# chaofengc/FeMaSR

Hardware: AMD Instinct MI355X
Metric: SR output megapixels/sec at x4 (128->512) (higher is better)
Workload: dtype f32 (1x1 convs / nn.Linear: every fp32 operand split EXACTLY into three bf16 terms, six partial products, fp32 accumulation on the bf16 matrix pipe - closer to fp64 than the fp32 fmaf chain, bit-identical to the CPU oracle)

## Files before the change

femasr_amd/csrc/kernels_misc.hip:

```cpp
#include "common.h"
#include "detmath.h"
#include <stdlib.h>
#include <string.h>

namespace {

__device__ __forceinline__ float4 ld4(const float *p) { return *reinterpret_cast<const float4 *>(p); }

__device__ __forceinline__ int xcd_remap_misc(int bid, int nblk)
{
    const int q = nblk >> 3, r = nblk & 7, xcd = bid & 7, within = bid >> 3;
    return (xcd < r ? xcd * (q + 1) : r * (q + 1) + (xcd - r) * q) + within;
}

__global__ void pad_nchw_to_nhwc_kernel(const float *__restrict__ in, int B, int C, int H, int W, int Hp, int Wp,
                                        float *__restrict__ out, size_t total)
{
    for (size_t i = blockIdx.x * (size_t)blockDim.x + threadIdx.x; i < total; i += (size_t)gridDim.x * blockDim.x) {
        const int c = (int)(i % C);
        size_t r = i / C;
        const int x = (int)(r % Wp);
        r /= Wp;
        const int y = (int)(r % Hp);
        const int n = (int)(r / Hp);
// ... 148 lines not shown
    const int slabs = C >> 5, cg = C >> 5;
    int b = blockIdx.x;
    const int slab = b % slabs;
    b /= slabs;
    const int tx = b % tilesX;
    b /= tilesX;
    const int ty = b % tilesY;
    const int n = b / tilesY;
    const float *xn = x + (size_t)n * H * W * C + slab * 32 + c31;
    double S = 0.0, SS = 0.0;
#pragma unroll
    for (int q = 0; q < 4; ++q) {
        double s = 0.0, ss = 0.0;
#pragma unroll
        for (int r = 0; r < 16; ++r) {
            const int m = 32 * q + 4 * h + (r & 3) + 8 * (r >> 2);
            const int y = 8 * ty + (m >> 4), xx = 16 * tx + (m & 15);
            if (y < H && xx < W) {
                const double d = (double)xn[((size_t)y * W + xx) * C];
                s = s + d;
                ss = __builtin_fma(d, d, ss);
            }
        }
        s = s + __shfl_xor(s, 32, 64);
        ss = ss + __shfl_xor(ss, 32, 64);
        for (int d = 1; d < cg; d <<= 1) {
            s = s + __shfl_xor(s, d, 64);
            ss = ss + __shfl_xor(ss, d, 64);
        }
        if (q == 0) { S = s; SS = ss; } else { S = S + s; SS = SS + ss; }
    }
    const int ch = slab * 32 + c31;
    if (lane < 32 && (ch & (cg - 1)) == 0) {
        double *dst = part + ((((size_t)n * tilesY + ty) * tilesX + tx) * 32 + ch / cg) * 2;
        dst[0] = S;
        dst[1] = SS;
    }
}

__global__ __launch_bounds__(64) void gn_finalize_partials_kernel(const double *__restrict__ part, int tiles, int H, int W, int C, int G,
                                                                  const float *__restrict__ gamma, const float *__restrict__ beta,
                                                                  float eps, float *__restrict__ a, float *__restrict__ b)
{
    const int n = blockIdx.x / G, g = blockIdx.x % G, lane = threadIdx.x, cg = C / G;
    const double *src = part + ((size_t)n * tiles * G + g) * 2;
    double S = 0.0, SS = 0.0;
    for (int t = lane; t < tiles; t += 64) {
        S += src[(size_t)t * G * 2];
        SS += src[(size_t)t * G * 2 + 1];
    }
#pragma unroll
    for (int sft = 32; sft >= 1; sft >>= 1) {
        S += __shfl_xor(S, sft, 64);
        SS += __shfl_xor(SS, sft, 64);
    }
    const double N = (double)H * (double)W * (double)cg;
    const double mean = S / N;
    double var = SS / N - mean * mean;
    if (var < 0.0) var = 0.0;
    const float rstd = 1.0f / sqrtf((float)var + eps);
    const float meanf = (float)mean;
    if (lane < cg) {
        const int c = g * cg + lane;
        const float ac = rstd * gamma[c];
        a[n * C + c] = ac;
        b[n * C + c] = __builtin_fmaf(-meanf, ac, beta[c]);
    }
}

__global__ void gn_silu_apply_kernel(const float *__restrict__ x, int C, long long hw, const float *__restrict__ a, const float *__restrict__ b,
                                     float *__restrict__ y, size_t total4)
{
    const int c4n = C >> 2;
    for (size_t i = blockIdx.x * (size_t)blockDim.x + threadIdx.x; i < total4; i += (size_t)gridDim.x * blockDim.x) {
        const int c4 = (int)(i % c4n);
        const size_t n = (i / c4n) / (size_t)hw;
        const float4 v = ld4(x + 4 * i), ga = ld4(a + n * C + 4 * c4), gb = ld4(b + n * C + 4 * c4);
        float4 o;
        o.x = det_silu(__builtin_fmaf(v.x, ga.x, gb.x));
        o.y = det_silu(__builtin_fmaf(v.y, ga.y, gb.y));
        o.z = det_silu(__builtin_fmaf(v.z, ga.z, gb.z));
        o.w = det_silu(__builtin_fmaf(v.w, ga.w, gb.w));
        *reinterpret_cast<float4 *>(y + 4 * i) = o;
    }
}

__device__ __forceinline__ float wave_tree_sum(float p)
{
#pragma unroll
    for (int s = 32; s >= 1; s >>= 1) p = p + __shfl_xor(p, s, 64);
    return p;
}

__global__ void ln_stats_kernel(const float *__restrict__ x, long long rows, float eps, float *__restrict__ stats)
{
    const long long row = (long long)blockIdx.x * (blockDim.x >> 6) + (threadIdx.x >> 6);
    if (row >= rows) return;
    const int lane = threadIdx.x & 63;
    const float4 v = ld4(x + row * 256 + lane * 4);
    float s = v.x;
    s = s + v.y;
    s = s + v.z;
    s = s + v.w;
    const float mean = wave_tree_sum(s) * (1.0f / 256.0f);
    float d = v.x - mean;
    float q = d * d;
    d = v.y - mean;
    q = __builtin_fmaf(d, d, q);
    d = v.z - mean;
    q = __builtin_fmaf(d, d, q);
    d = v.w - mean;
    q = __builtin_fmaf(d, d, q);
    const float var = wave_tree_sum(q) * (1.0f / 256.0f);
    if (lane == 0) {
        stats[2 * row] = mean;
        stats[2 * row + 1] = 1.0f / sqrtf(var + eps);
    }
}

__global__ void layernorm_kernel(const float *__restrict__ x, long long rows, const float *__restrict__ gamma,
                                 const float *__restrict__ beta, float eps, float *__restrict__ y)
{
    const long long row = (long long)blockIdx.x * (blockDim.x >> 6) + (threadIdx.x >> 6);
    if (row >= rows) return;
    const int lane = threadIdx.x & 63;
    const float4 v = ld4(x + row * 256 + lane * 4);
    float s = v.x;
    s = s + v.y;
    s = s + v.z;
    s = s + v.w;
    const float mean = wave_tree_sum(s) * (1.0f / 256.0f);
    float d = v.x - mean;
    float q = d * d;
    d = v.y - mean;
    q = __builtin_fmaf(d, d, q);
    d = v.z - mean;
    q = __builtin_fmaf(d, d, q);
    d = v.w - mean;
    q = __builtin_fmaf(d, d, q);
    const float var = wave_tree_sum(q) * (1.0f / 256.0f);
    const float rstd = 1.0f / sqrtf(var + eps);
    const float4 g = ld4(gamma + lane * 4), b = ld4(beta + lane * 4);
    float4 o;
    o.x = __builtin_fmaf((v.x - mean) * rstd, g.x, b.x);
    o.y = __builtin_fmaf((v.y - mean) * rstd, g.y, b.y);
    o.z = __builtin_fmaf((v.z - mean) * rstd, g.z, b.z);
    o.w = __builtin_fmaf((v.w - mean) * rstd, g.w, b.w);
    *reinterpret_cast<float4 *>(y + row * 256 + lane * 4) = o;
}

constexpr int ATT_HD = 32, ATT_N = 64;
typedef float att_f32x16 __attribute__((ext_vector_type(16)));

template <int UNITS>
__global__ __launch_bounds__(64, 2) void window_attention_reg_kernel(const float *__restrict__ qkv, int B, int H, int W, int C,
                                                                     int heads, int shift, const float *__restrict__ table,
                                                                     float *__restrict__ out, int total)
{
    __shared__ float Ts[UNITS][232];
    const int lane = threadIdx.x, c = lane & 31, hf = lane >> 5;
    const int nwx = W >> 3, nwy = H >> 3;
    struct Unit { int h, wx, wy, n; };
    auto unit_of = [&](int bid) {
        Unit g;
        g.h = bid % heads;
        bid /= heads;
        g.wx = bid % nwx;
        bid /= nwx;
        g.wy = bid % nwy;
        g.n = bid / nwy;
        return g;
    };
    Unit gs[UNITS];
    bool has[UNITS];
#pragma unroll
    for (int u = 0; u < UNITS; ++u) {
        const int bid = (int)blockIdx.x * UNITS + u;
        has[u] = bid < total;
        gs[u] = unit_of(has[u] ? bid : total - 1);
        for (int i = lane; i < 225; i += 64) Ts[u][i] = table[i * heads + gs[u].h];
    }
    const float scale = 0.17677669529663687f;
    auto rowtok = [&](const Unit &g, int iy) { int y = g.wy * 8 + iy + shift; if (y >= H) y -= H; return y * W; };
    auto coltok = [&](const Unit &g, int ix) { int x = g.wx * 8 + ix + shift; if (x >= W) x -= W; return x; };
    auto qb = [&](const Unit &g) { return qkv + (size_t)g.n * H * W * 3 * C + g.h * ATT_HD; };

    float ak[2][16], bq[2][16];
    auto load_qk = [&](const Unit &g) {
        const float *qbase = qb(g);
#pragma unroll
        for (int tI = 0; tI < 2; ++tI) {
            const int w = 32 * tI + c;
            const unsigned tok = (unsigned)(rowtok(g, w >> 3) + coltok(g, w & 7));
            const float *kp = qbase + tok * (unsigned)(3 * C) + C, *qp = qbase + tok * (unsigned)(3 * C);
#pragma unroll
            for (int d4 = 0; d4 < 8; ++d4) {
                const float4 kv = ld4(kp + 4 * d4), qv = ld4(qp + 4 * d4);
                ak[tI][2 * d4] = hf ? kv.y : kv.x;
                ak[tI][2 * d4 + 1] = hf ? kv.w : kv.z;
                bq[tI][2 * d4] = (hf ? qv.y : qv.x) * scale;
                bq[tI][2 * d4 + 1] = (hf ? qv.w : qv.z) * scale;
            }
        }
    };
    load_qk(gs[0]);
#pragma unroll
    for (int u = 0; u < UNITS; ++u) {
        if (!has[u]) break;
        const Unit g = gs[u];
        const float *qbase = qb(g);
        float *obase = out + (size_t)g.n * H * W * C + g.h * ATT_HD;
        const bool masked = shift > 0 && (g.wy == nwy - 1 || g.wx == nwx - 1);
        att_f32x16 sc[2][2];
#pragma unroll
        for (int tj = 0; tj < 2; ++tj)
#pragma unroll
            for (int ti = 0; ti < 2; ++ti)
#pragma unroll
                for (int r = 0; r < 16; ++r) sc[tj][ti][r] = 0.f;
#pragma unroll
        for (int st = 0; st < 16; ++st)
#pragma unroll
            for (int tj = 0; tj < 2; ++tj)
#pragma unroll
                for (int ti = 0; ti < 2; ++ti) sc[tj][ti] = __builtin_amdgcn_mfma_f32_32x32x2f32(ak[tj][st], bq[ti][st], sc[tj][ti], 0, 0, 0);

        float vf[2][16];
        {
            const float *vb = qbase + 2 * C + c;
            unsigned cto[4];
#pragma unroll
            for (int e = 0; e < 4; ++e) cto[e] = (unsigned)coltok(g, e + 4 * hf) * (unsigned)(3 * C);
#pragma unroll
            for (int tj = 0; tj < 2; ++tj)
#pragma unroll
                for (int r = 0; r < 16; ++r) {
                    const unsigned ro = (unsigned)__builtin_amdgcn_readfirstlane(rowtok(g, (r >> 2) + 4 * tj)) * (unsigned)(3 * C);
                    vf[tj][r] = vb[ro + cto[r & 3]];
                }
        }
        if (u + 1 < UNITS && has[u + 1 < UNITS ? u + 1 : u]) load_qk(gs[u + 1 < UNITS ? u + 1 : u]);
#pragma unroll
        for (int ti = 0; ti < 2; ++ti) {
            const int i = 32 * ti + c, iy = i >> 3, ix = i & 7;
            const int tb = (iy + 7) * 15 + ix + 7 - 4 * hf;
            unsigned rowdiff = 0, coldiff = 0;
            if (masked) {
                const int ysi = g.wy * 8 + iy, xsi = g.wx * 8 + ix;
                const int ryi = ysi < H - 8 ? 0 : (ysi < H - shift ? 1 : 2), rxi = xsi < W - 8 ? 0 : (xsi < W - shift ? 1 : 2);
#pragma unroll
                for (int q = 0; q < 8; ++q) {
                    const int ysj = g.wy * 8 + q, xsj = g.wx * 8 + q;
                    const int ryj = ysj < H - 8 ? 0 : (ysj < H - shift ? 1 : 2), rxj = xsj < W - 8 ? 0 : (xsj < W - shift ? 1 : 2);
                    rowdiff |= (ryj != ryi ? 1u : 0u) << q;
                    coldiff |= (rxj != rxi ? 1u : 0u) << q;
                }
                coldiff >>= 4 * hf;
            }
            float m = -INFINITY;
#pragma unroll
            for (int tj = 0; tj < 2; ++tj)
#pragma unroll
                for (int r = 0; r < 16; ++r) {
                    const int jy = (r >> 2) + 4 * tj, jxl = r & 3;
                    float a1 = sc[tj][ti][r] + Ts[u][tb - 15 * jy - jxl];
                    if (masked) a1 = a1 + ((((rowdiff >> jy) | (coldiff >> jxl)) & 1u) ? -100.0f : 0.0f);
                    sc[tj][ti][r] = a1;
                    m = a1 > m ? a1 : m;
                }
            {
                const float mo = __shfl_xor(m, 32, 64);
                m = mo > m ? mo : m;
            }
            float part = 0.f;
#pragma unroll
            for (int tj = 0; tj < 2; ++tj)
#pragma unroll
                for (int r = 0; r < 16; r += 2) {
                    const det_f32x2 e = det_expf2(det_f32x2{sc[tj][ti][r] - m, sc[tj][ti][r + 1] - m});
                    sc[tj][ti][r] = e[0];
                    sc[tj][ti][r + 1] = e[1];
                    part = part + e[0];
                    part = part + e[1];
                }
            const float other = __shfl_xor(part, 32, 64);
            const float rinv = 1.0f / (hf ? other + part : part + other);
#pragma unroll
            for (int tj = 0; tj < 2; ++tj) sc[tj][ti] = sc[tj][ti] * rinv;
        }

        att_f32x16 oc[2];
#pragma unroll
        for (int ti = 0; ti < 2; ++ti)
#pragma unroll
            for (int r = 0; r < 16; ++r) oc[ti][r] = 0.f;
#pragma unroll
        for (int tj = 0; tj < 2; ++tj)
#pragma unroll
            for (int r = 0; r < 16; ++r)
#pragma unroll
                for (int ti = 0; ti < 2; ++ti) oc[ti] = __builtin_amdgcn_mfma_f32_32x32x2f32(sc[tj][ti][r], vf[tj][r], oc[ti], 0, 0, 0);

        {
            float *ob = obase + c;
            unsigned cto[4];
#pragma unroll
            for (int e = 0; e < 4; ++e) cto[e] = (unsigned)coltok(g, e + 4 * hf) * (unsigned)C;
#pragma unroll
            for (int ti = 0; ti < 2; ++ti)
#pragma unroll
                for (int r = 0; r < 16; ++r) {
                    const unsigned ro = (unsigned)__builtin_amdgcn_readfirstlane(rowtok(g, (r >> 2) + 4 * ti)) * (unsigned)C;
                    ob[ro + cto[r & 3]] = oc[ti][r];
                }
        }
    }
}

__global__ void row_sqsum_kernel(const float *__restrict__ x, long long rows, int D, float *__restrict__ out)
{
    const long long r = (long long)blockIdx.x * blockDim.x + threadIdx.x;
    if (r >= rows) return;
    const float *p = x + r * D;
    float acc = 0.f;
    for (int c = 0; c < D; c += 4) {
        const float4 v = ld4(p + c);
        acc = __builtin_fmaf(v.x, v.x, acc);
        acc = __builtin_fmaf(v.y, v.y, acc);
        acc = __builtin_fmaf(v.z, v.z, acc);
        acc = __builtin_fmaf(v.w, v.w, acc);
    }
    out[r] = acc;
}

__global__ void vq_finalize_kernel(const float *__restrict__ z, long long M, int D, const float *__restrict__ cb,
                                   const float *__restrict__ part, int nblk, int n_e, long long *__restrict__ idx,
                                   float *__restrict__ zq)
{
    const long long row = (long long)blockIdx.x * (blockDim.x >> 6) + (threadIdx.x >> 6);
    if (row >= M) return;
    const int lane = threadIdx.x & 63;
    const float *pp = part + (size_t)row * nblk * 2;
    float bd = pp[0];
    int bi = __float_as_int(pp[1]);
    for (int b = 1; b < nblk; ++b) {
        const float d = pp[2 * b];
        const int i = __float_as_int(pp[2 * b + 1]);
        if (d < bd || (d == bd && i < bi)) { bd = d; bi = i; }
    }
    bi = bi < 0 ? 0 : (bi >= n_e ? n_e - 1 : bi);
    if (lane == 0) idx[row] = (long long)bi;
    const float *e = cb + (size_t)bi * D;
    const float *zr = z + (size_t)row * D;
    float *o = zq + (size_t)row * D;
    for (int c = lane * 4; c < D; c += 256) {
        const float4 zv = ld4(zr + c), ev = ld4(e + c);
        float4 r;
        r.x = zv.x + (ev.x - zv.x);
        r.y = zv.y + (ev.y - zv.y);
        r.z = zv.z + (ev.z - zv.z);
        r.w = zv.w + (ev.w - zv.w);
        *reinterpret_cast<float4 *>(o + c) = r;
    }
}

__global__ void codebook_gather_kernel(const long long *__restrict__ idx, long long M, int D, const float *__restrict__ cb,
                                       int n_e, float *__restrict__ zq)
{
    const long long row = (long long)blockIdx.x * (blockDim.x >> 6) + (threadIdx.x >> 6);
    if (row >= M) return;
    const int lane = threadIdx.x & 63;
    long long i = idx[row];
    i = i < 0 ? 0 : (i >= n_e ? n_e - 1 : i);
    for (int c = lane * 4; c < D; c += 256)
        *reinterpret_cast<float4 *>(zq + (size_t)row * D + c) = ld4(cb + (size_t)i * D + c);
}

__global__ void repack_oihw_kernel(const float *__restrict__ in, int O, int I, int kh, int kw, float *__restrict__ out,
                                   size_t total)
{
    const bool blocked = (I % 32) == 0;
    const int K = I * kh * kw, NT32 = (O + 31) / 32;
    for (size_t i = blockIdx.x * (size_t)blockDim.x + threadIdx.x; i < total; i += (size_t)gridDim.x * blockDim.x) {
        const int kk = (int)(i & 15), lane = (int)((i >> 4) & 63);
        const size_t rest = i >> 10;
        const int ntile = (int)(rest % NT32), q = (int)(rest / NT32);
        const int k = q * 32 + kk * 2 + (lane >> 5), o = ntile * 32 + (lane & 31);
        float v = 0.f;
        if (k < K && o < O) {
            int ci, x, y;
            if (blocked) {
                const int cl = k % 32;
                int r = k / 32;
                x = r % kw;
                r /= kw;
                y = r % kh;
                ci = (r / kh) * 32 + cl;
            } else {
                ci = k % I;
                const int r = k / I;
                x = r % kw;
                y = r / kw;
            }
            v = in[(((size_t)o * I + ci) * kh + y) * kw + x];
        }
        out[i] = v;
    }
}

__global__ void repack_up2_kernel(const float *__restrict__ in, int O, int I, float *__restrict__ out, size_t per_phase)
{
    const int K = I * 4, NT32 = (O + 31) / 32;
    for (size_t i = blockIdx.x * (size_t)blockDim.x + threadIdx.x; i < 4 * per_phase; i += (size_t)gridDim.x * blockDim.x) {
        const int ph = (int)(i / per_phase);
        const size_t e = i - (size_t)ph * per_phase;
        const int kk = (int)(e & 15), lane = (int)((e >> 4) & 63);
        const size_t rest = e >> 10;
        const int ntile = (int)(rest % NT32), q = (int)(rest / NT32);
        const int k = q * 32 + kk * 2 + (lane >> 5), o = ntile * 32 + (lane & 31);
        float v = 0.f;
        if (k < K && o < O) {
            const int a = ph >> 1, b = ph & 1;
            const int cl = k % 32, r = k / 32, tap = r & 3, ci = (r >> 2) * 32 + cl;
            const int ty = tap >> 1, tx = tap & 1;
            const int y0 = ty == 0 ? 0 : (a == 0 ? 1 : 2), y1 = ty == 0 ? (a == 0 ? 0 : 1) : 2;
            const int x0 = tx == 0 ? 0 : (b == 0 ? 1 : 2), x1 = tx == 0 ? (b == 0 ? 0 : 1) : 2;
            const float *w = in + ((size_t)o * I + ci) * 9;
            for (int ky = y0; ky <= y1; ++ky) {
                float row = w[ky * 3 + x0];
                for (int kx = x0 + 1; kx <= x1; ++kx) row = row + w[ky * 3 + kx];
                v = ky == y0 ? row : v + row;
            }
        }
        out[i] = v;
    }
}

__global__ void repack_compact_kernel(const float *__restrict__ in, int O, int I, int kh, int kw, float *__restrict__ out, size_t total)
{
    for (size_t i = blockIdx.x * (size_t)blockDim.x + threadIdx.x; i < total; i += (size_t)gridDim.x * blockDim.x) {
        const int o = (int)(i & 3), k = (int)(i >> 2);
        const int cl = k % 32;
        int r = k / 32;
        const int x = r % kw;
        r /= kw;
        const int y = r % kh, ci = (r / kh) * 32 + cl;
        out[i] = o < O ? in[(((size_t)o * I + ci) * kh + y) * kw + x] : 0.f;
    }
}

__global__ void image_u8_to_f32_kernel(const unsigned char *__restrict__ in, int H, int W, int swap_rb,
                                       float *__restrict__ out, size_t total)
{
    for (size_t i = blockIdx.x * (size_t)blockDim.x + threadIdx.x; i < total; i += (size_t)gridDim.x * blockDim.x) {
        const int x = (int)(i % W);
        size_t r = i / W;
        const int y = (int)(r % H);
        const int c = (int)(r / H);
        const int sc = swap_rb ? 2 - c : c;
        out[i] = (float)in[((size_t)y * W + x) * 3 + sc] / 255.0f;
    }
}

__global__ void image_f32_to_u8_kernel(const float *__restrict__ in, int H, int W, int swap_rb,
                                       unsigned char *__restrict__ out, size_t total)
{
    for (size_t i = blockIdx.x * (size_t)blockDim.x + threadIdx.x; i < total; i += (size_t)gridDim.x * blockDim.x) {
// ... 100 lines not shown
}

typedef float probe_f32x16 __attribute__((ext_vector_type(16)));
__global__ __launch_bounds__(256) void clock_probe_kernel(int groups, float a, float b, unsigned long long *ticks)
{
    probe_f32x16 c0 = {0}, c1 = {0}, c2 = {0}, c3 = {0};
    a += (float)(threadIdx.x & 31) * 0.03125f;
    b += (float)((threadIdx.x >> 5) & 1) * 0.25f;
    const unsigned long long t0 = __builtin_readcyclecounter();
    for (int i = 0; i < groups; ++i) {
        c0 = __builtin_amdgcn_mfma_f32_32x32x2f32(a, b, c0, 0, 0, 0);
        c1 = __builtin_amdgcn_mfma_f32_32x32x2f32(a, b, c1, 0, 0, 0);
        c2 = __builtin_amdgcn_mfma_f32_32x32x2f32(a, b, c2, 0, 0, 0);
        c3 = __builtin_amdgcn_mfma_f32_32x32x2f32(a, b, c3, 0, 0, 0);
    }
    float s = 0.f;
    for (int r = 0; r < 16; ++r) s += c0[r] + c1[r] + c2[r] + c3[r];
    const unsigned long long t1 = __builtin_readcyclecounter();
    if ((threadIdx.x & 63) == 0) ticks[blockIdx.x * 4 + (threadIdx.x >> 6)] = (t1 - t0) + (s == 12345.678f ? 1ull : 0ull);
}

extern "C" {

int femasr_pad_nchw_to_nhwc(void *stream, const float *in, int B, int C, int H, int W, int Hp, int Wp, float *out)
{
    FEMASR_REQUIRE(in && out && B > 0 && C > 0 && H > 0 && W > 0, "pad: bad args");
    FEMASR_REQUIRE(Hp >= H && Wp >= W && Hp - H <= H && Wp - W <= W, "pad: mirror pad larger than the image (%d,%d)->(%d,%d)", H, W, Hp, Wp);
    const size_t total = (size_t)B * Hp * Wp * C;
    hipLaunchKernelGGL(pad_nchw_to_nhwc_kernel, dim3(grid_for(total)), dim3(256), 0, (hipStream_t)stream, in, B, C, H, W,
                       Hp, Wp, out, total);
    FEMASR_CHECK_HIP(hipGetLastError());
    return FEMASR_OK;
}

int femasr_pad_u8hwc_to_nhwc(void *stream, const uint8_t *in, int B, int H, int W, int swap_rb, int Hp, int Wp, float *out)
{
    FEMASR_REQUIRE(in && out && B > 0 && H > 0 && W > 0 && Hp >= H && Wp >= W && Hp <= 2 * H && Wp <= 2 * W, "pad_u8: bad args");
    const size_t total = (size_t)B * Hp * Wp * 3;
    hipLaunchKernelGGL(pad_u8hwc_to_nhwc_kernel, dim3(grid_for(total)), dim3(256), 0, (hipStream_t)stream, in, B, H, W, swap_rb, Hp, Wp, out, total);
    FEMASR_CHECK_HIP(hipGetLastError());
    return FEMASR_OK;
}

int femasr_crop_nhwc_to_u8hwc(void *stream, const float *in, int B, int Hs, int Ws, int Hc, int Wc, int swap_rb, uint8_t *out)
{
    FEMASR_REQUIRE(in && out && B > 0 && Hc > 0 && Wc > 0 && Hc <= Hs && Wc <= Ws, "crop_u8: bad args");
    const size_t total = (size_t)B * Hc * Wc * 3;
    hipLaunchKernelGGL(crop_nhwc_to_u8hwc_kernel, dim3(grid_for(total)), dim3(256), 0, (hipStream_t)stream, in, B, Hs, Ws, Hc, Wc, swap_rb, out, total);
    FEMASR_CHECK_HIP(hipGetLastError());
    return FEMASR_OK;
}

int femasr_crop_nhwc_to_nchw(void *stream, const float *in, int B, int Hs, int Ws, int C, int Hc, int Wc, float *out)
{
    FEMASR_REQUIRE(in && out && B > 0 && C > 0 && Hc > 0 && Wc > 0 && Hc <= Hs && Wc <= Ws, "crop: bad args");
    const size_t total = (size_t)B * C * Hc * Wc;
    hipLaunchKernelGGL(crop_nhwc_to_nchw_kernel, dim3(grid_for(total)), dim3(256), 0, (hipStream_t)stream, in, B, Hs, Ws,
                       C, Hc, Wc, out, total);
    FEMASR_CHECK_HIP(hipGetLastError());
    return FEMASR_OK;
}

size_t femasr_gn_scratch_bytes(int B, int H, int W, int C, int G)
{
    if (B <= 0 || H <= 0 || W <= 0 || G <= 0) return 0;
    if (G == 32 && femasr_gn_fusable(C)) return (size_t)B * ((H + 7) / 8) * ((W + 15) / 16) * 32 * 2 * sizeof(double);
    return (size_t)B * H * G * 2 * sizeof(double);
}

int femasr_gn_coeffs(void *stream, const float *x, int B, int H, int W, int C, int G, const float *gamma,
                     const float *beta, float eps, float *a, float *b, void *scratch)
{
    FEMASR_REQUIRE(x && gamma && beta && a && b && scratch, "gn_coeffs: null pointer");
    FEMASR_REQUIRE(B > 0 && H > 0 && W > 0 && G > 0 && C % G == 0, "gn_coeffs: bad shape C=%d G=%d", C, G);
    const int cg = C / G;
    hipStream_t s = (hipStream_t)stream;
    double *part = (double *)scratch;
    if (G == 32 && femasr_gn_fusable(C)) {
        const int tilesX = (W + 15) / 16, tilesY = (H + 7) / 8;
        hipLaunchKernelGGL(gn_tile_partials_kernel, dim3((unsigned)((size_t)B * tilesY * tilesX * (C / 32))), dim3(64), 0, s, x, H, W, C,
                           tilesX, tilesY, part);
        FEMASR_CHECK_HIP(hipGetLastError());
        return femasr_gn_coeffs_from_partials(stream, part, B, tilesX * tilesY, H, W, C, G, gamma, beta, eps, a, b);
    }
    const size_t total = (size_t)B * H * G;
    const dim3 grid((unsigned)((total + 255) / 256)), blk(256);
    if (cg == 8 && C % 4 == 0)
        hipLaunchKernelGGL(gn_rows_kernel<8>, grid, blk, 0, s, x, B, H, W, C, G, part);
    else if (cg == 4 && C % 4 == 0)
        hipLaunchKernelGGL(gn_rows_kernel<4>, grid, blk, 0, s, x, B, H, W, C, G, part);
    else if (cg == 2)
        hipLaunchKernelGGL(gn_rows_kernel<2>, grid, blk, 0, s, x, B, H, W, C, G, part);
    else
        hipLaunchKernelGGL(gn_rows_generic_kernel, grid, blk, 0, s, x, B, H, W, C, G, cg, part);
    FEMASR_CHECK_HIP(hipGetLastError());
    FEMASR_REQUIRE(G <= 256, "gn_coeffs: at most 256 groups");
    hipLaunchKernelGGL(gn_finalize_kernel, dim3((unsigned)B), dim3(256), (size_t)GN_SLAB * G * 2 * sizeof(double), s, part, B, H, H,
                       W, C, G, gamma, beta, eps, a, b);
    FEMASR_CHECK_HIP(hipGetLastError());
    return FEMASR_OK;
}

int femasr_gn_coeffs_from_partials(void *stream, const double *part, int B, int tiles, int H, int W, int C, int G,
                                   const float *gamma, const float *beta, float eps, float *a, float *b)
{
    FEMASR_REQUIRE(part && gamma && beta && a && b && B > 0 && tiles > 0 && H > 0 && W > 0, "gn_coeffs_from_partials: bad args");
    FEMASR_REQUIRE(G == 32 && C % G == 0, "gn_coeffs_from_partials: 32 groups");
    FEMASR_REQUIRE(C / G <= 64, "gn_coeffs_from_partials: at most 64 channels per group");
    hipLaunchKernelGGL(gn_finalize_partials_kernel, dim3((unsigned)(B * G)), dim3(64), 0, (hipStream_t)stream, part, tiles, H, W, C,
                       G, gamma, beta, eps, a, b);
    FEMASR_CHECK_HIP(hipGetLastError());
    return FEMASR_OK;
}

int femasr_gn_silu_apply(void *stream, const float *x, int B, int H, int W, int C, const float *a, const float *b, float *y)
{
    FEMASR_REQUIRE(x && a && b && y && B > 0 && H > 0 && W > 0 && C > 0 && (C % 4) == 0, "gn_silu_apply: bad args (C %% 4 == 0)");
    const size_t total4 = (size_t)B * H * W * (C / 4);
    hipLaunchKernelGGL(gn_silu_apply_kernel, dim3(grid_for(total4)), dim3(256), 0, (hipStream_t)stream, x, C, (long long)H * W, a, b, y, total4);
    FEMASR_CHECK_HIP(hipGetLastError());
    return FEMASR_OK;
}

int femasr_ln_stats(void *stream, const float *x, int64_t rows, int C, float eps, float *stats)
{
    FEMASR_REQUIRE(x && stats && rows > 0, "ln_stats: bad args");
    FEMASR_REQUIRE(C == 256, "ln_stats: only C == 256 (Swin embed_dim, femasr_arch.py:115) is built, got %d", C);
    hipLaunchKernelGGL(ln_stats_kernel, dim3((unsigned)((rows + 3) / 4)), dim3(256), 0, (hipStream_t)stream, x,
                       (long long)rows, eps, stats);
    FEMASR_CHECK_HIP(hipGetLastError());
    return FEMASR_OK;
}

int femasr_layernorm(void *stream, const float *x, int64_t rows, int C, const float *gamma, const float *beta, float eps, float *y)
{
    FEMASR_REQUIRE(x && y && gamma && beta && rows > 0, "layernorm: bad args");
    FEMASR_REQUIRE(C == 256, "layernorm: only C == 256 (Swin embed_dim, femasr_arch.py:115) is built, got %d", C);
    hipLaunchKernelGGL(layernorm_kernel, dim3((unsigned)((rows + 3) / 4)), dim3(256), 0, (hipStream_t)stream, x, (long long)rows,
                       gamma, beta, eps, y);
    FEMASR_CHECK_HIP(hipGetLastError());
    return FEMASR_OK;
}

int femasr_window_attention(void *stream, const float *qkv, int B, int H, int W, int C, int heads, int shift,
                            const float *table, float *out)
{
    FEMASR_REQUIRE(qkv && table && out && B > 0, "window_attention: bad args");
    FEMASR_REQUIRE(H % 8 == 0 && W % 8 == 0 && H >= 8 && W >= 8, "window_attention: H,W must be multiples of 8 (%d,%d)", H, W);
    FEMASR_REQUIRE(heads > 0 && heads <= 8 && C == heads * ATT_HD, "window_attention: head_dim must be 32, at most 8 heads (C=%d heads=%d)", C, heads);
    FEMASR_REQUIRE(shift >= 0 && shift < 8, "window_attention: bad shift %d", shift);
    FEMASR_REQUIRE((size_t)H * W * 3 * C < ((size_t)1 << 30), "window_attention: image too large for 32-bit offsets");
    const size_t total = (size_t)B * (H / 8) * (W / 8) * heads;
    FEMASR_REQUIRE(total < ((size_t)1 << 31), "window_attention: too many (window, head) units");
    static const int units = [] { const char *e = getenv("FEMASR_ATT_UNITS"); return (e && atoi(e) == 2) ? 2 : 1; }();
    if (units == 2)
        hipLaunchKernelGGL(window_attention_reg_kernel<2>, dim3((unsigned)((total + 1) / 2)), dim3(64), 0, (hipStream_t)stream, qkv, B, H, W, C, heads,
                           shift, table, out, (int)total);
    else
        hipLaunchKernelGGL(window_attention_reg_kernel<1>, dim3((unsigned)total), dim3(64), 0, (hipStream_t)stream, qkv, B, H, W, C, heads, shift, table,
                           out, (int)total);
    FEMASR_CHECK_HIP(hipGetLastError());
    return FEMASR_OK;
}

int femasr_row_sqsum(void *stream, const float *x, int64_t rows, int D, float *out)
{
    FEMASR_REQUIRE(x && out && rows > 0 && D > 0 && D % 4 == 0, "row_sqsum: bad args");
    hipLaunchKernelGGL(row_sqsum_kernel, dim3((unsigned)((rows + 63) / 64)), dim3(64), 0, (hipStream_t)stream, x,
                       (long long)rows, D, out);
    FEMASR_CHECK_HIP(hipGetLastError());
    return FEMASR_OK;
}

int femasr_vq(void *stream, const float *z, int64_t M, int D, const float *cb, const float *cbT, const float *ee,
              int n_e, int64_t *idx, float *zq, void *scratch)
{
    FEMASR_REQUIRE(z && cb && cbT && ee && idx && zq && scratch && M > 0, "vq: bad args");
    FEMASR_REQUIRE(D % 32 == 0 && n_e % 128 == 0, "vq: needs e_dim %% 32 == 0 and n_e %% 128 == 0 (D=%d n_e=%d)", D, n_e);
    FEMASR_REQUIRE(M < (1ll << 31) - 256, "vq: too many rows");
    hipStream_t s = (hipStream_t)stream;
    float *zz = (float *)scratch;
    float *part = zz + ((M + 63) / 64) * 64;
    const int nblk = n_e / 128;
    int rc = femasr_row_sqsum(stream, z, M, D, zz);
    if (rc) return rc;
    femasr_conv_args a{};
    a.in = z; a.B = 1; a.H = (int)M; a.W = 1; a.Cin = D; a.w = cbT; a.bias = nullptr; a.Cout = n_e;
    a.ksz = 1; a.stride = 1; a.pad = 0; a.up2 = 0; a.prologue = FEMASR_PRO_NONE; a.act = 0;
    a.Ho = (int)M; a.Wo = 1;
    conv_vq_epilogue ep{zz, ee, part, nblk};
    rc = femasr_conv2d_launch(s, &a, &ep, nullptr, nullptr);
    if (rc) return rc;
    hipLaunchKernelGGL(vq_finalize_kernel, dim3((unsigned)((M + 3) / 4)), dim3(256), 0, s, z, (long long)M, D, cb, part,
                       nblk, n_e, (long long *)idx, zq);
    FEMASR_CHECK_HIP(hipGetLastError());
    return FEMASR_OK;
}

int femasr_codebook_gather(void *stream, const int64_t *idx, int64_t M, int D, const float *cb, int n_e, float *zq)
{
    FEMASR_REQUIRE(idx && cb && zq && M > 0 && D % 4 == 0 && n_e > 0, "codebook_gather: bad args");
    hipLaunchKernelGGL(codebook_gather_kernel, dim3((unsigned)((M + 3) / 4)), dim3(256), 0, (hipStream_t)stream,
                       (const long long *)idx, (long long)M, D, cb, n_e, zq);
    FEMASR_CHECK_HIP(hipGetLastError());
    return FEMASR_OK;
}

int femasr_extract_tiles(void *stream, const float *in, int B, int C, int H, int W, const int32_t *yx_dev, int n, int th, int tw, float *out)
{
    FEMASR_REQUIRE(in && yx_dev && out && B > 0 && C > 0 && n > 0 && th > 0 && tw > 0 && th <= H && tw <= W, "extract_tiles: bad args");
    const size_t total = (size_t)n * B * C * th * tw;
    hipLaunchKernelGGL(extract_tiles_kernel, dim3(grid_for(total)), dim3(256), 0, (hipStream_t)stream, in, B, C, H, W, yx_dev, n, th, tw, out, total);
    FEMASR_CHECK_HIP(hipGetLastError());
    return FEMASR_OK;
}

int femasr_paste_tiles(void *stream, const float *tiles, int B, int C, int n, int th, int tw, const int32_t *rects_dev, int hmax,
                       int Ho, int Wo, float *out)
{
    FEMASR_REQUIRE(tiles && rects_dev && out && B > 0 && C > 0 && n > 0 && th > 0 && tw > 0 && hmax > 0 && hmax <= th, "paste_tiles: bad args");
    const size_t rows = (size_t)n * B * C * hmax;
    FEMASR_REQUIRE(rows < ((size_t)1 << 31), "paste_tiles: too many rows");
    hipLaunchKernelGGL(paste_tiles_kernel, dim3((unsigned)rows), dim3(256), 0, (hipStream_t)stream, tiles, B, C, th, tw, rects_dev, n, Ho, Wo, out, hmax);
    FEMASR_CHECK_HIP(hipGetLastError());
    return FEMASR_OK;
}

int femasr_extract_tiles_u8(void *stream, const uint8_t *in, int B, int H, int W, const int32_t *yx_dev, int n, int th, int tw, uint8_t *out)
{
    FEMASR_REQUIRE(in && yx_dev && out && B > 0 && n > 0 && th > 0 && tw > 0 && th <= H && tw <= W, "extract_tiles_u8: bad args");
    const size_t total = (size_t)n * B * th * tw * 3;
    hipLaunchKernelGGL(extract_tiles_u8_kernel, dim3(grid_for(total)), dim3(256), 0, (hipStream_t)stream, in, B, H, W, yx_dev, n, th, tw, out, total);
    FEMASR_CHECK_HIP(hipGetLastError());
    return FEMASR_OK;
}

int femasr_paste_tiles_u8(void *stream, const uint8_t *tiles, int B, int n, int th, int tw, const int32_t *rects_dev, int hmax, int Ho, int Wo, uint8_t *out)
{
    FEMASR_REQUIRE(tiles && rects_dev && out && B > 0 && n > 0 && th > 0 && tw > 0 && hmax > 0 && hmax <= th, "paste_tiles_u8: bad args");
    const size_t rows = (size_t)n * B * hmax;
    FEMASR_REQUIRE(rows < ((size_t)1 << 31), "paste_tiles_u8: too many rows");
    hipLaunchKernelGGL(paste_tiles_u8_kernel, dim3((unsigned)rows), dim3(256), 0, (hipStream_t)stream, tiles, B, th, tw, rects_dev, n, Ho, Wo, out, hmax);
    FEMASR_CHECK_HIP(hipGetLastError());
    return FEMASR_OK;
}

int femasr_concat_resize(void *stream, const float *a, int Ca, const float *b, int Hb, int Wb, int Cb, int B, int H, int W, float *out)
{
    FEMASR_REQUIRE(a && b && out && B > 0 && H > 0 && W > 0 && Hb > 0 && Wb > 0, "concat_resize: bad args");
    FEMASR_REQUIRE(Ca > 0 && Cb > 0 && Ca % 4 == 0 && Cb % 4 == 0, "concat_resize: channel counts must be multiples of 4 (%d, %d)", Ca, Cb);
    const size_t total4 = (size_t)B * H * W * ((Ca + Cb) / 4);
    hipLaunchKernelGGL(concat_resize_kernel, dim3(grid_for(total4)), dim3(256), 0, (hipStream_t)stream, a, Ca, b, Hb, Wb, Cb, H, W, out,
                       total4);
    FEMASR_CHECK_HIP(hipGetLastError());
    return FEMASR_OK;
}

size_t femasr_packed_weight_floats(int O, int I, int kh, int kw)
{
    if (O <= 0 || I <= 0 || kh <= 0 || kw <= 0) return 0;
    const size_t K = (size_t)I * kh * kw;
    return ((K + 31) / 32) * (size_t)((O + 31) / 32) * 1024 + femasr_compact_weight_floats(O, I, kh, kw);
}

int femasr_repack_oihw(void *stream, const float *in, int O, int I, int kh, int kw, float *out)
{
    FEMASR_REQUIRE(in && out && O > 0 && I > 0 && kh > 0 && kw > 0, "repack: bad args");
    if (kh == 1 && kw == 1 && (I % 32) == 0) return femasr_repack_k1((hipStream_t)stream, in, O, I, out);
    const size_t tail = femasr_compact_weight_floats(O, I, kh, kw);
    const size_t total = femasr_packed_weight_floats(O, I, kh, kw) - tail;
    if (tail) {
        hipLaunchKernelGGL(repack_compact_kernel, dim3(grid_for(tail)), dim3(256), 0, (hipStream_t)stream, in, O, I, kh, kw, out + total, tail);
        FEMASR_CHECK_HIP(hipGetLastError());
    }
    hipLaunchKernelGGL(repack_oihw_kernel, dim3(grid_for(total)), dim3(256), 0, (hipStream_t)stream, in, O, I, kh, kw, out,
                       total);
    FEMASR_CHECK_HIP(hipGetLastError());
    return FEMASR_OK;
}

size_t femasr_up2_weight_floats(int O, int I)
{
    return (I % 32) == 0 ? 4 * femasr_packed_weight_floats(O, I, 2, 2) : 0;
}

int femasr_repack_oihw_up2(void *stream, const float *in, int O, int I, float *out)
{
    FEMASR_REQUIRE(in && out && O > 0 && I > 0 && (I % 32) == 0, "repack_up2: needs a 3x3 OIHW weight with I %% 32 == 0");
    const size_t per = femasr_packed_weight_floats(O, I, 2, 2);
    hipLaunchKernelGGL(repack_up2_kernel, dim3(grid_for(4 * per)), dim3(256), 0, (hipStream_t)stream, in, O, I, out, per);
    FEMASR_CHECK_HIP(hipGetLastError());
    return FEMASR_OK;
}

int femasr_image_u8_to_f32(void *stream, const uint8_t *in_hwc, int H, int W, int swap_rb, float *out_chw)
{
    FEMASR_REQUIRE(in_hwc && out_chw && H > 0 && W > 0, "image_u8_to_f32: bad args");
    const size_t total = (size_t)3 * H * W;
    hipLaunchKernelGGL(image_u8_to_f32_kernel, dim3(grid_for(total)), dim3(256), 0, (hipStream_t)stream, in_hwc, H, W,
                       swap_rb, out_chw, total);
    FEMASR_CHECK_HIP(hipGetLastError());
    return FEMASR_OK;
}

int femasr_image_f32_to_u8(void *stream, const float *in_chw, int H, int W, int swap_rb, uint8_t *out_hwc)
{
    FEMASR_REQUIRE(in_chw && out_hwc && H > 0 && W > 0, "image_f32_to_u8: bad args");
    const size_t total = (size_t)3 * H * W;
    hipLaunchKernelGGL(image_f32_to_u8_kernel, dim3(grid_for(total)), dim3(256), 0, (hipStream_t)stream, in_chw, H, W,
                       swap_rb, out_hwc, total);
    FEMASR_CHECK_HIP(hipGetLastError());
    return FEMASR_OK;
}
// ... 87 lines not shown
```

Baseline: 68.63.

## Restructure window attention to process query tiles sequentially and cut registers

The window attention kernel now handles one window-head per block and loops over the two 32-row query tiles one after another, so it keeps a single score pair and a single output accumulator instead of the full 2x2 score set. Launch bounds rise from 2 to 3 waves per SIMD. Q/K rows are now loaded as contiguous float4s and redistributed across half-waves with permlane32_swap instead of the old strided per-half selects. The goal is lower register pressure and higher occupancy to better hide memory latency. The cost is serialised softmax work per tile and the removal of the optional two-unit prefetch path.

```diff
diff --git a/femasr_amd/csrc/kernels_misc.hip b/femasr_amd/csrc/kernels_misc.hip
--- a/femasr_amd/csrc/kernels_misc.hip
+++ b/femasr_amd/csrc/kernels_misc.hip
@@ -324,105 +324,96 @@
 constexpr int ATT_HD = 32, ATT_N = 64;
 typedef float att_f32x16 __attribute__((ext_vector_type(16)));
 
-template <int UNITS>
-__global__ __launch_bounds__(64, 2) void window_attention_reg_kernel(const float *__restrict__ qkv, int B, int H, int W, int C,
+__global__ __launch_bounds__(64, 3) void window_attention_reg_kernel(const float *__restrict__ qkv, int B, int H, int W, int C,
                                                                      int heads, int shift, const float *__restrict__ table,
-                                                                     float *__restrict__ out, int total)
-{
-    __shared__ float Ts[UNITS][232];
+                                                                     float *__restrict__ out)
+{
+    __shared__ float Ts[232];
     const int lane = threadIdx.x, c = lane & 31, hf = lane >> 5;
     const int nwx = W >> 3, nwy = H >> 3;
-    struct Unit { int h, wx, wy, n; };
-    auto unit_of = [&](int bid) {
-        Unit g;
-        g.h = bid % heads;
-        bid /= heads;
-        g.wx = bid % nwx;
-        bid /= nwx;
-        g.wy = bid % nwy;
-        g.n = bid / nwy;
-        return g;
+    int bid = (int)blockIdx.x;
+    const int gh = bid % heads;
+    bid /= heads;
+    const int gwx = bid % nwx;
+    bid /= nwx;
+    const int gwy = bid % nwy, gn = bid / nwy;
+    for (int i = lane; i < 225; i += 64) Ts[i] = table[i * heads + gh];
+    const float scale = 0.17677669529663687f;
+    auto rowtok = [&](int iy) { int y = gwy * 8 + iy + shift; if (y >= H) y -= H; return y * W; };
+    auto coltok = [&](int ix) { int x = gwx * 8 + ix + shift; if (x >= W) x -= W; return x; };
+    const float *qbase = qkv + (size_t)gn * H * W * 3 * C + gh * ATT_HD;
+    float *obase = out + (size_t)gn * H * W * C + gh * ATT_HD;
+
+    auto load_row = [&](const float *base, int t, float (&dst)[16]) {
+        const int w = 32 * t + c;
+        const unsigned tok = (unsigned)(rowtok(w >> 3) + coltok(w & 7));
+        const float *p = reinterpret_cast<const float *>(reinterpret_cast<const char *>(base) + (tok * (unsigned)(3 * C) + 16u * hf) * 4u);
+        float r[16];
+#pragma unroll
+        for (int q4 = 0; q4 < 4; ++q4) {
+            const float4 v = ld4(p + 4 * q4);
+            r[4 * q4] = v.x;
+            r[4 * q4 + 1] = v.y;
+            r[4 * q4 + 2] = v.z;
+            r[4 * q4 + 3] = v.w;
+        }
+#pragma unroll
+        for (int m = 0; m < 8; ++m) {
+            const auto sw = __builtin_amdgcn_permlane32_swap(__float_as_uint(r[2 * m]), __float_as_uint(r[2 * m + 1]), false, false);
+            dst[m] = __uint_as_float(sw[0]);
+            dst[8 + m] = __uint_as_float(sw[1]);
+        }
     };
-    Unit gs[UNITS];
-    bool has[UNITS];
-#pragma unroll
-    for (int u = 0; u < UNITS; ++u) {
-        const int bid = (int)blockIdx.x * UNITS + u;
-        has[u] = bid < total;
-        gs[u] = unit_of(has[u] ? bid : total - 1);
-        for (int i = lane; i < 225; i += 64) Ts[u][i] = table[i * heads + gs[u].h];
-    }
-    const float scale = 0.17677669529663687f;
-    auto rowtok = [&](const Unit &g, int iy) { int y = g.wy * 8 + iy + shift; if (y >= H) y -= H; return y * W; };
-    auto coltok = [&](const Unit &g, int ix) { int x = g.wx * 8 + ix + shift; if (x >= W) x -= W; return x; };
-    auto qb = [&](const Unit &g) { return qkv + (size_t)g.n * H * W * 3 * C + g.h * ATT_HD; };
-
-    float ak[2][16], bq[2][16];
-    auto load_qk = [&](const Unit &g) {
-        const float *qbase = qb(g);
-#pragma unroll
-        for (int tI = 0; tI < 2; ++tI) {
-            const int w = 32 * tI + c;
-            const unsigned tok = (unsigned)(rowtok(g, w >> 3) + coltok(g, w & 7));
-            const float *kp = qbase + tok * (unsigned)(3 * C) + C, *qp = qbase + tok * (unsigned)(3 * C);
-#pragma unroll
-            for (int d4 = 0; d4 < 8; ++d4) {
-                const float4 kv = ld4(kp + 4 * d4), qv = ld4(qp + 4 * d4);
-                ak[tI][2 * d4] = hf ? kv.y : kv.x;
-                ak[tI][2 * d4 + 1] = hf ? kv.w : kv.z;
-                bq[tI][2 * d4] = (hf ? qv.y : qv.x) * scale;
-                bq[tI][2 * d4 + 1] = (hf ? qv.w : qv.z) * scale;
+    float ak[2][16];
+    load_row(qbase + C, 0, ak[0]);
+    load_row(qbase + C, 1, ak[1]);
+    const bool masked = shift > 0 && (gwy == nwy - 1 || gwx == nwx - 1);
+    float vf[2][16];
+#pragma unroll 1
+    for (int ti = 0; ti < 2; ++ti) {
+        float bq[16];
+        load_row(qbase, ti, bq);
+#pragma unroll
+        for (int st = 0; st < 16; ++st) bq[st] = bq[st] * scale;
+        att_f32x16 sc[2];
+#pragma unroll
+        for (int tj = 0; tj < 2; ++tj)
+#pragma unroll
+            for (int r = 0; r < 16; ++r) sc[tj][r] = 0.f;
+#pragma unroll
+        for (int st = 0; st < 16; ++st)
+#pragma unroll
+            for (int tj = 0; tj < 2; ++tj) sc[tj] = __builtin_amdgcn_mfma_f32_32x32x2f32(ak[tj][st], bq[st], sc[tj], 0, 0, 0);
+
+        if (ti == 0) {
+            const char *vb = reinterpret_cast<const char *>(qbase + 2 * C);
+            unsigned cto[4];
+#pragma unroll
+            for (int e = 0; e < 4; ++e) {
+                cto[e] = ((unsigned)coltok(e + 4 * hf) * (unsigned)(3 * C) + c) * 4u;
+                asm("" : "+v"(cto[e]));
             }
-        }
-    };
-    load_qk(gs[0]);
-#pragma unroll
-    for (int u = 0; u < UNITS; ++u) {
-        if (!has[u]) break;
-        const Unit g = gs[u];
-        const float *qbase = qb(g);
-        float *obase = out + (size_t)g.n * H * W * C + g.h * ATT_HD;
-        const bool masked = shift > 0 && (g.wy == nwy - 1 || g.wx == nwx - 1);
-        att_f32x16 sc[2][2];
-#pragma unroll
-        for (int tj = 0; tj < 2; ++tj)
-#pragma unroll
-            for (int ti = 0; ti < 2; ++ti)
-#pragma unroll
-                for (int r = 0; r < 16; ++r) sc[tj][ti][r] = 0.f;
-#pragma unroll
-        for (int st = 0; st < 16; ++st)
 #pragma unroll
             for (int tj = 0; tj < 2; ++tj)
 #pragma unroll
-                for (int ti = 0; ti < 2; ++ti) sc[tj][ti] = __builtin_amdgcn_mfma_f32_32x32x2f32(ak[tj][st], bq[ti][st], sc[tj][ti], 0, 0, 0);
-
-        float vf[2][16];
+                for (int r4 = 0; r4 < 4; ++r4) {
+                    unsigned ro = (unsigned)__builtin_amdgcn_readfirstlane(rowtok(r4 + 4 * tj)) * (unsigned)(3 * C);
+                    asm("" : "+s"(ro));
+                    const char *vrow = vb + (size_t)ro * 4;
+#pragma unroll
+                    for (int e = 0; e < 4; ++e) vf[tj][4 * r4 + e] = *reinterpret_cast<const float *>(vrow + cto[e]);
+                }
+        }
         {
-            const float *vb = qbase + 2 * C + c;
-            unsigned cto[4];
-#pragma unroll
-            for (int e = 0; e < 4; ++e) cto[e] = (unsigned)coltok(g, e + 4 * hf) * (unsigned)(3 * C);
-#pragma unroll
-            for (int tj = 0; tj < 2; ++tj)
-#pragma unroll
-                for (int r = 0; r < 16; ++r) {
-                    const unsigned ro = (unsigned)__builtin_amdgcn_readfirstlane(rowtok(g, (r >> 2) + 4 * tj)) * (unsigned)(3 * C);
-                    vf[tj][r] = vb[ro + cto[r & 3]];
-                }
-        }
-        if (u + 1 < UNITS && has[u + 1 < UNITS ? u + 1 : u]) load_qk(gs[u + 1 < UNITS ? u + 1 : u]);
-#pragma unroll
-        for (int ti = 0; ti < 2; ++ti) {
             const int i = 32 * ti + c, iy = i >> 3, ix = i & 7;
             const int tb = (iy + 7) * 15 + ix + 7 - 4 * hf;
             unsigned rowdiff = 0, coldiff = 0;
             if (masked) {
-                const int ysi = g.wy * 8 + iy, xsi = g.wx * 8 + ix;
+                const int ysi = gwy * 8 + iy, xsi = gwx * 8 + ix;
                 const int ryi = ysi < H - 8 ? 0 : (ysi < H - shift ? 1 : 2), rxi = xsi < W - 8 ? 0 : (xsi < W - shift ? 1 : 2);
 #pragma unroll
                 for (int q = 0; q < 8; ++q) {
-                    const int ysj = g.wy * 8 + q, xsj = g.wx * 8 + q;
+                    const int ysj = gwy * 8 + q, xsj = gwx * 8 + q;
                     const int ryj = ysj < H - 8 ? 0 : (ysj < H - shift ? 1 : 2), rxj = xsj < W - 8 ? 0 : (xsj < W - shift ? 1 : 2);
                     rowdiff |= (ryj != ryi ? 1u : 0u) << q;
                     coldiff |= (rxj != rxi ? 1u : 0u) << q;
@@ -431,15 +422,17 @@
             }
             float m = -INFINITY;
 #pragma unroll
-            for (int tj = 0; tj < 2; ++tj)
+            for (int tj = 0; tj < 2; ++tj) {
+                if (tj) asm volatile("" ::: "memory");
 #pragma unroll
                 for (int r = 0; r < 16; ++r) {
                     const int jy = (r >> 2) + 4 * tj, jxl = r & 3;
-                    float a1 = sc[tj][ti][r] + Ts[u][tb - 15 * jy - jxl];
+                    float a1 = sc[tj][r] + Ts[tb - 15 * jy - jxl];
                     if (masked) a1 = a1 + ((((rowdiff >> jy) | (coldiff >> jxl)) & 1u) ? -100.0f : 0.0f);
-                    sc[tj][ti][r] = a1;
+                    sc[tj][r] = a1;
                     m = a1 > m ? a1 : m;
                 }
+            }
             {
                 const float mo = __shfl_xor(m, 32, 64);
                 m = mo > m ? mo : m;
@@ -449,42 +442,42 @@
             for (int tj = 0; tj < 2; ++tj)
 #pragma unroll
                 for (int r = 0; r < 16; r += 2) {
-                    const det_f32x2 e = det_expf2(det_f32x2{sc[tj][ti][r] - m, sc[tj][ti][r + 1] - m});
-                    sc[tj][ti][r] = e[0];
-                    sc[tj][ti][r + 1] = e[1];
+                    const det_f32x2 e = det_expf2(det_f32x2{sc[tj][r] - m, sc[tj][r + 1] - m});
+                    sc[tj][r] = e[0];
+                    sc[tj][r + 1] = e[1];
                     part = part + e[0];
                     part = part + e[1];
                 }
             const float other = __shfl_xor(part, 32, 64);
             const float rinv = 1.0f / (hf ? other + part : part + other);
 #pragma unroll
-            for (int tj = 0; tj < 2; ++tj) sc[tj][ti] = sc[tj][ti] * rinv;
-        }
-
-        att_f32x16 oc[2];
-#pragma unroll
-        for (int ti = 0; ti < 2; ++ti)
-#pragma unroll
-            for (int r = 0; r < 16; ++r) oc[ti][r] = 0.f;
+            for (int tj = 0; tj < 2; ++tj) sc[tj] = sc[tj] * rinv;
+        }
+
+        att_f32x16 oc;
+#pragma unroll
+        for (int r = 0; r < 16; ++r) oc[r] = 0.f;
 #pragma unroll
         for (int tj = 0; tj < 2; ++tj)
 #pragma unroll
-            for (int r = 0; r < 16; ++r)
-#pragma unroll
-                for (int ti = 0; ti < 2; ++ti) oc[ti] = __builtin_amdgcn_mfma_f32_32x32x2f32(sc[tj][ti][r], vf[tj][r], oc[ti], 0, 0, 0);
+            for (int r = 0; r < 16; ++r) oc = __builtin_amdgcn_mfma_f32_32x32x2f32(sc[tj][r], vf[tj][r], oc, 0, 0, 0);
 
         {
-            float *ob = obase + c;
+            char *ob = reinterpret_cast<char *>(obase);
             unsigned cto[4];
 #pragma unroll
-            for (int e = 0; e < 4; ++e) cto[e] = (unsigned)coltok(g, e + 4 * hf) * (unsigned)C;
-#pragma unroll
-            for (int ti = 0; ti < 2; ++ti)
-#pragma unroll
-                for (int r = 0; r < 16; ++r) {
-                    const unsigned ro = (unsigned)__builtin_amdgcn_readfirstlane(rowtok(g, (r >> 2) + 4 * ti)) * (unsigned)C;
-                    ob[ro + cto[r & 3]] = oc[ti][r];
-                }
+            for (int e = 0; e < 4; ++e) {
+                cto[e] = ((unsigned)coltok(e + 4 * hf) * (unsigned)C + c) * 4u;
+                asm("" : "+v"(cto[e]));
+            }
+#pragma unroll
+            for (int r4 = 0; r4 < 4; ++r4) {
+                unsigned ro = (unsigned)__builtin_amdgcn_readfirstlane(rowtok(r4 + 4 * ti)) * (unsigned)C;
+                asm("" : "+s"(ro));
+                char *orow = ob + (size_t)ro * 4;
+#pragma unroll
+                for (int e = 0; e < 4; ++e) *reinterpret_cast<float *>(orow + cto[e]) = oc[4 * r4 + e];
+            }
         }
     }
 }
@@ -891,13 +884,8 @@
     FEMASR_REQUIRE((size_t)H * W * 3 * C < ((size_t)1 << 30), "window_attention: image too large for 32-bit offsets");
     const size_t total = (size_t)B * (H / 8) * (W / 8) * heads;
     FEMASR_REQUIRE(total < ((size_t)1 << 31), "window_attention: too many (window, head) units");
-    static const int units = [] { const char *e = getenv("FEMASR_ATT_UNITS"); return (e && atoi(e) == 2) ? 2 : 1; }();
-    if (units == 2)
-        hipLaunchKernelGGL(window_attention_reg_kernel<2>, dim3((unsigned)((total + 1) / 2)), dim3(64), 0, (hipStream_t)stream, qkv, B, H, W, C, heads,
-                           shift, table, out, (int)total);
-    else
-        hipLaunchKernelGGL(window_attention_reg_kernel<1>, dim3((unsigned)total), dim3(64), 0, (hipStream_t)stream, qkv, B, H, W, C, heads, shift, table,
-                           out, (int)total);
+    hipLaunchKernelGGL(window_attention_reg_kernel, dim3((unsigned)total), dim3(64), 0, (hipStream_t)stream, qkv, B, H, W, C, heads,
+                       shift, table, out);
     FEMASR_CHECK_HIP(hipGetLastError());
     return FEMASR_OK;
 }
```

Result: no change. 69.14 (median of 6 runs) (+0.7%).
